# balazs-bamer/cdpr-simulation

Hardware: AMD Instinct MI355X
Metric: CDPR sim-steps/sec (whole node), 65 536 parallel 8-cable robots, 1 ms dt (higher is better)
Workload: dtype f32

## Files before the change

cdpr-simulation_amd/csrc/cdpr_onestep_kernel.hpp:

```cpp
#pragma once
#include "cdpr_step_kernel.hpp"

namespace cdpr {

CDPR_DEV void row_to_lds(const float4* src, float4* dst_row) {
  __builtin_amdgcn_global_load_lds((const __attribute__((address_space(1))) void*)src, (__attribute__((address_space(3))) void*)dst_row, 16, 0, 0);
}


template <int NP, bool PR = false, bool FULL = false>
CDPR_DEV void pid_pairs(const StepArgs& a, int calls, bool is_vel, const v2f (&desired)[NP], const v2f (&actual)[NP], const v2f (&win)[NP][kWin],
                        v2f (&ierr)[NP], v2f (&f)[NP], v2f (&e_new)[NP], float& dbg_p, float& dbg_i, float& dbg_d, bool is_force = false) {
  const PidCoef c = pid_coef<PR>(a, is_vel);
  const bool run = (!PR || calls != 0) && !is_force;
  const bool full = FULL || calls >= c.nbuf;
  const float (&wt)[kWin + 2] = a.wrow;
  v2f error[NP], acc[NP];
#pragma unroll
  for (int k = 0; k < NP; ++k) {
    error[k] = desired[k] - actual[k];
    acc[k] = splat(wt[kWin]) * error[k];
  }
#pragma unroll
  for (int j = 0; j < kWin; ++j) {
// ... 228 lines not shown
      ierr[2 * g] = (v2f){h.x, h.y};
      if (2 * g + 1 < NP) ierr[2 * g + 1] = (v2f){h.z, h.w};
    }
    const bool actual_is_vel = (a.flags & kFlagActualIsVelocity) != 0u;
    v2f actual[NP];
#pragma unroll
    for (int k = 0; k < NP; ++k) actual[k] = actual_is_vel ? qd[k] : q[k];
    const int ring_slot = a.ring_slot;
    pid_pairs<NP>(a, a.pid_calls, actual_is_vel, desired, actual, win, ierr, f, e_new, dbg_p, dbg_i, dbg_d);
    dbg_wrote = true;
    if (live) {
#pragma unroll
      for (int m = 0; m < 5; ++m) {
        if (m == (ring_slot >> 1)) {
#pragma unroll
          for (int k = 0; k < NP; ++k) CDPR_STORE_STATE(a.state, st, P + 5 * k + m, woff, ring_row(win[k], m, e_new[k], ring_slot));
        }
      }
#pragma unroll
      for (int g = 0; g < NH; ++g) {
        const int k1 = (2 * g + 1 < NP) ? 2 * g + 1 : 2 * g;
        CDPR_STORE_STATE(a.state, st, P + 5 * NP + g, woff, make_float4(ierr[2 * g].x, ierr[2 * g].y, ierr[k1].x, ierr[k1].y));
      }
    }
  }

  if (force_mode && !first_world) {
#pragma unroll
    for (int k = 0; k < NP; ++k) f[k] = desired[k];
  }

  if (PERSIST && more) {
    const uint32_t noff = nrr * 16u;
    if (run_pid) {
#pragma unroll
      for (int j = 0; j < kCtrl; ++j)
        row_to_lds(reinterpret_cast<const float4*>(reinterpret_cast<const char*>(a.state + (size_t)(P + j) * st) + noff), &stage[j][0]);
      if (kCmdLds) {
        const float* ncp = a.cmd + (size_t)nrr * N;
#pragma unroll
        for (int g = 0; g < kCmdRows; ++g) row_to_lds(reinterpret_cast<const float4*>(ncp) + g, &stage[kCtrl + g][0]);
      }
    }
  }

  CDPR_STAMP(5);
  v2f applied[NP];
  int td_flag = 0;
  if (TD) {
    v2f df[NP];
#pragma unroll
    for (int k = 0; k < NP; ++k) df[k] = f[k] - splat(a.td_mid);
    float g[6];
    if (FK) {
      jt_times<NP>(jest, df, g);
      normal_solve<NP, false>(jest, 0.f, g);
    } else {
      jt_times<NP>(jac, df, g);
      normal_solve<NP, false>(jac, 0.f, g);
    }
#pragma unroll
    for (int k = 0; k < NP; ++k) {
      v2f t = splat(a.td_mid);
#pragma unroll
      for (int c = 0; c < 6; ++c) t = fma2(g[c], FK ? jest[k][c] : jac[k][c], t);
      const v2f tc = max2(min2(t, splat(a.td_max)), splat(a.td_min));
      td_flag |= (tc.x != t.x) ? 1 : 0;
      if (2 * k + 1 < N) td_flag |= (tc.y != t.y) ? 1 : 0;
      applied[k] = tc;
    }
  } else {
#pragma unroll
    for (int k = 0; k < NP; ++k) applied[k] = f[k];
  }
  setforce_limits<NP>(a, qd, applied);

  if (a.dbg && live) write_pid_topic(a.dbg + (size_t)r * 9, dbg_wrote, dbg_wrote, dbg_p, dbg_i, dbg_d, desired[0].x, applied[0].x);
  if (publish && live) {
    store_slot(a.obs, st, 3, woff, make_float4(s.wz, fk_res, (float)fk_it, pack_flags(td_flag, travel_mask<N>(a, q))));
#pragma unroll
    for (int g = 0; g < G; ++g) {
      const int k0 = 2 * g, k1 = (2 * g + 1 < NP) ? 2 * g + 1 : 2 * g;
      const bool has = (2 * g + 1 < NP);
      store_slot(a.obs, st, 4 + 2 * G + g, woff,
                make_float4(applied[k0].x, applied[k0].y, has ? applied[k1].x : 0.f, has ? applied[k1].y : 0.f));
    }
  }

  CDPR_STAMP(6);
  {
    v2f tens[NP];
#pragma unroll
    for (int k = 0; k < NP; ++k) {
      tens[k] = fma2(-a.damping, qd[k], applied[k]);
      if (a.unilateral) tens[k] = max2(tens[k], splat(0.f));
    }
    if (FK) {
      uint32_t again = 0;
      asm volatile("" : "+v"(again));
      v2f len2[NP], l02[NP];
      ik_pairs<N, false>(lds + again, s.px, s.py, s.pz, s.qx, s.qy, s.qz, s.qw, len2, jac, l02);
    }
    float w[6];
    jt_times<NP>(jac, tens, w);
    w[0] = a.fgx - w[0];
    w[1] = a.fgy - w[1];
    w[2] = a.fgz - w[2];
    w[3] = -w[3];
    w[4] = -w[4];
    w[5] = -w[5];
    integrate(a, s, w);
  }
  if (PERSIST && more) {
    constexpr int kDmaOps = kCtrl + kCmdRows;
    static_assert(kDmaOps < 64, "vmcnt is a 6-bit counter");
    if (run_pid)
      __builtin_amdgcn_s_waitcnt(vmcnt_imm(kDmaOps));
    else
      __builtin_amdgcn_s_waitcnt(vmcnt_imm(0));
    asm volatile("" : "+a"(n0), "+a"(n1), "+a"(n2), "+a"(n3), "+a"(n4));
  }
  if (live) {
    CDPR_STORE_STATE(a.state, st, 0, woff, make_float4(s.px, s.py, s.pz, s.qx));
    CDPR_STORE_STATE(a.state, st, 1, woff, make_float4(s.qy, s.qz, s.qw, s.vx));
    CDPR_STORE_STATE(a.state, st, 2, woff, make_float4(s.vy, s.vz, s.wx, s.wy));
    CDPR_STORE_STATE(a.state, st, 3, woff, make_float4(s.wz, fkx, fky, fkz));
    if (FK) CDPR_STORE_STATE(a.state, st, 4, woff, make_float4(fkqx, fkqy, fkqz, fkqw));
  }
  CDPR_STAMP(7);
  if (!(PERSIST && more)) break;
  blk = nblk;
  r = nr;
  rr = nrr;
  live = r < a.batch;
  off = rr * 16u, woff = r * 16u;
  p0 = make_float4(n0.x, n0.y, n0.z, n0.w), p1 = make_float4(n1.x, n1.y, n1.z, n1.w), p2 = make_float4(n2.x, n2.y, n2.z, n2.w);
  p3 = make_float4(n3.x, n3.y, n3.z, n3.w), p4 = make_float4(n4.x, n4.y, n4.z, n4.w);
  staged = run_pid;
  }
}

#ifndef CDPR_CTL_LOAD_DELAY
#define CDPR_CTL_LOAD_DELAY 8
#endif
#ifndef CDPR_SPLIT_PRIO
#define CDPR_SPLIT_PRIO 1
#endif
#ifndef CDPR_STEADY_SHARED_IK
#define CDPR_STEADY_SHARED_IK 1
#endif
#ifndef CDPR_STEADY_NEWTON_WRITTEN_OUT
#define CDPR_STEADY_NEWTON_WRITTEN_OUT 1
#endif
constexpr int kIkRows = 7;
#ifdef CDPR_STAMPS
#define CDPR_SPLIT_STAMP(i)                                                                                          \
  do {                                                                                                               \
    __builtin_amdgcn_sched_barrier(0);                                                                               \
    if (a.stamps && lane == 0) a.stamps[(size_t)blockIdx.x * 8 + (i)] = __builtin_amdgcn_s_memrealtime();           \
    __builtin_amdgcn_sched_barrier(0);                                                                               \
  } while (0)
#else
#define CDPR_SPLIT_STAMP(i) do { } while (0)
#endif
#if defined(CDPR_STAMPS) && defined(CDPR_STAMPS_ITER)
#define CDPR_CTL_STAMP(i) do { } while (0)
#else
#define CDPR_CTL_STAMP(i) CDPR_SPLIT_STAMP(i)
#endif

template <int N, int XS, int ES, bool RAISED = true, bool STEADY = false>
CDPR_DEV void split_estimator_wave(const StepArgs& a, float* geo, float gval, uint32_t lane, bool live, size_t st, uint32_t off, uint32_t woff,
                                   const float4& p0, const float4& p1, const float4& p3, const v2f* x_force, v2f* x_tension, float* x_est,
                                   v2f* x_ik = nullptr) {
  constexpr int NP = cable_pairs(N);
#if defined(CDPR_STAMPS) && defined(CDPR_STAMPS_CLOCK)
  const unsigned long long clk0 = __builtin_amdgcn_s_memtime();
#endif
#if CDPR_SPLIT_PRIO == 1 || CDPR_SPLIT_PRIO == 4
  if (RAISED) __builtin_amdgcn_s_setprio(3);
#elif CDPR_SPLIT_PRIO == 3 || CDPR_SPLIT_PRIO == 5
  if (RAISED) __builtin_amdgcn_s_setprio(2);
#endif
  const float4 p4 = load_slot(a.state, st, 4, off);
  if (lane < NP * kGeomFloatsPerPair) geo[lane] = gval;
  __builtin_amdgcn_fence(__ATOMIC_RELEASE, "wavefront");
  __builtin_amdgcn_wave_barrier();
  __builtin_amdgcn_fence(__ATOMIC_ACQUIRE, "wavefront");
  float fkx = p3.y, fky = p3.z, fkz = p3.w, fkqx = p4.x, fkqy = p4.y, fkqz = p4.z, fkqw = p4.w;
  v2f len[NP];
  {
    v2f jac[NP][6], l0[NP];
    ik_pairs<N, false>(geo, p0.x, p0.y, p0.z, p0.w, p1.x, p1.y, p1.z, len, jac, l0);
    if (STEADY && CDPR_STEADY_SHARED_IK) {
#pragma unroll
      for (int k = 0; k < NP; ++k) {
        x_ik[(kIkRows * k) * 64 + lane] = len[k];
#pragma unroll
        for (int c = 0; c < 6; ++c) x_ik[(kIkRows * k + 1 + c) * 64 + lane] = jac[k][c];
      }
      __builtin_amdgcn_fence(__ATOMIC_RELEASE, "workgroup");
      __builtin_amdgcn_s_waitcnt(0xC07F);
      __builtin_amdgcn_s_barrier();
    }
  }
  float fk_res = 0.f;
  int fk_it = 0;
  v2f jest[NP][6];
  {
    v2f elen[NP], unused[NP];
    if (STEADY && CDPR_STEADY_NEWTON_WRITTEN_OUT) {
#pragma unroll
      for (int it = 0; it < 4; ++it) {
        ik_pairs<N, false>(geo, fkx, fky, fkz, fkqx, fkqy, fkqz, fkqw, elen, jest, unused);
        v2f res[NP];
#pragma unroll
        for (int k = 0; k < NP; ++k) res[k] = len[k] - elen[k];
        float g[6];
        jt_times<NP>(jest, res, g);
        normal_solve<NP>(jest, a.fk_lambda, g);
        fkx += g[0];
        fky += g[1];
        fkz += g[2];
        quat_apply_rotvec(fkqx, fkqy, fkqz, fkqw, g[3], g[4], g[5]);
#ifdef CDPR_STAMPS_ITER
        if (it < 3) {
          asm volatile("" ::"v"(fkqw));
          __builtin_amdgcn_sched_barrier(0);
          if (a.stamps && lane == 0) a.stamps[(size_t)blockIdx.x * 8 + 4 + it] = __builtin_amdgcn_s_memrealtime();
          __builtin_amdgcn_sched_barrier(0);
        }
#endif
      }
      fk_it = 4;
    } else {
      bool active = true;
      for (int it = 0; it < a.fk_iters; ++it) {
        ik_pairs<N, false>(geo, fkx, fky, fkz, fkqx, fkqy, fkqz, fkqw, elen, jest, unused);
        v2f res[NP];
        v2f rm = splat(0.f);
#pragma unroll
        for (int k = 0; k < NP; ++k) {
          res[k] = len[k] - elen[k];
          rm = max2(rm, abs2(res[k]));
        }
        active = active && !(fmaxf(rm.x, rm.y) < a.fk_tol);
        float g[6];
        jt_times<NP>(jest, res, g);
        normal_solve<NP>(jest, a.fk_lambda, g);
        if (active) {
          fkx += g[0];
          fky += g[1];
          fkz += g[2];
          quat_apply_rotvec(fkqx, fkqy, fkqz, fkqw, g[3], g[4], g[5]);
          ++fk_it;
        }
#ifdef CDPR_STAMPS_ITER
        if (it < 3) {
          asm volatile("" ::"v"(fkqw));
          __builtin_amdgcn_sched_barrier(0);
          if (a.stamps && lane == 0) a.stamps[(size_t)blockIdx.x * 8 + 4 + it] = __builtin_amdgcn_s_memrealtime();
          __builtin_amdgcn_sched_barrier(0);
        }
#endif
      }
    }
    ik_pairs<N, false>(geo, fkx, fky, fkz, fkqx, fkqy, fkqz, fkqw, elen, jest, unused);
    v2f rm = splat(0.f);
#pragma unroll
    for (int k = 0; k < NP; ++k) rm = max2(rm, abs2(len[k] - elen[k]));
    fk_res = fmaxf(rm.x, rm.y);
  }
  if (live) store_slot_aux<CDPR_SPLIT_PLAT_AUX>(a.state, st, 4, woff, make_float4(fkqx, fkqy, fkqz, fkqw));
  CDPR_SPLIT_STAMP(1);
  v2f td_l[6][3];
  float td_invd[6];
  normal_matrix_pk<NP, false>(jest, 0.f, td_l);
  chol_factor_pk(td_l, td_invd);
  __builtin_amdgcn_s_waitcnt(0xC07F);
  __builtin_amdgcn_s_barrier();
  CDPR_SPLIT_STAMP(2);
  __builtin_amdgcn_fence(__ATOMIC_ACQUIRE, "workgroup");
  v2f f[NP], df[NP], t_out[NP];
#pragma unroll
  for (int k = 0; k < NP; ++k) {
    f[k] = x_force[k * XS + lane];
    df[k] = f[k] - splat(a.td_mid);
  }
  int td_flag = 0;
  {
    float g[6];
    jt_times<NP>(jest, df, g);
    chol_apply_pk(td_l, td_invd, g);
#pragma unroll
    for (int k = 0; k < NP; ++k) {
      v2f t = splat(a.td_mid);
#pragma unroll
      for (int c = 0; c < 6; ++c) t = fma2(g[c], jest[k][c], t);
      const v2f tc = max2(min2(t, splat(a.td_max)), splat(a.td_min));
      td_flag |= (tc.x != t.x) ? 1 : 0;
      if (2 * k + 1 < N) td_flag |= (tc.y != t.y) ? 1 : 0;
      t_out[k] = tc;
    }
  }
#pragma unroll
  for (int k = 0; k < NP; ++k) x_tension[k * XS + lane] = t_out[k];
  x_est[0 * ES + lane] = fkx;
  x_est[1 * ES + lane] = fky;
  x_est[2 * ES + lane] = fkz;
  x_est[3 * ES + lane] = fk_res;
  x_est[4 * ES + lane] = (float)fk_it;
  x_est[5 * ES + lane] = (float)td_flag;
  __builtin_amdgcn_fence(__ATOMIC_RELEASE, "workgroup");
  __builtin_amdgcn_s_waitcnt(0xC07F);
  CDPR_SPLIT_STAMP(3);
#if defined(CDPR_STAMPS) && defined(CDPR_STAMPS_CLOCK)
  if (a.stamps && lane == 0) a.stamps[(size_t)blockIdx.x * 8 + 7] = __builtin_amdgcn_s_memtime() - clk0;
#endif
  __builtin_amdgcn_s_barrier();
}

template <int N, bool PR, bool STEADY, bool VEL>
CDPR_DEV void split_controller_wave(const StepArgs& a, float* geo, float gval, uint32_t lane, uint32_t r, uint32_t rr, bool live, size_t st, uint32_t off,
                                    uint32_t woff, const float4& p0, const float4& p1, const float4& p2, const float4& p3, v2f* x_force, const v2f* x_tension,
                                    const float* x_est, const v2f* x_ik = nullptr) {
  static_assert(!(STEADY && PR), "the steady instantiation serves uniform handles");
  constexpr int NP = cable_pairs(N);
  constexpr int P = plat_slots(true);
  constexpr int G = joint_groups(N);
  constexpr int NH = (NP + 1) / 2;
#if CDPR_SPLIT_PRIO == 2 || CDPR_SPLIT_PRIO == 5
  __builtin_amdgcn_s_setprio(3);
#endif
#if CDPR_CTL_LOAD_DELAY > 0
  __builtin_amdgcn_s_sleep(CDPR_CTL_LOAD_DELAY);
#endif
  float4 wraw[NP][5], hraw[NH];
#pragma unroll
  for (int k = 0; k < NP; ++k) {
#pragma unroll
    for (int m = 0; m < 5; ++m) wraw[k][m] = load_slot(a.state, st, P + 5 * k + m, off);
  }
#pragma unroll
  for (int g = 0; g < NH; ++g) hraw[g] = load_slot(a.state, st, P + 5 * NP + g, off);
  v2f desired[NP];
#pragma unroll
  for (int k = 0; k < NP; ++k) desired[k] = splat(0.f);
  const float* cp = a.cmd + (size_t)rr * N;
  if (N % 4 == 0) {
#pragma unroll
    for (int g = 0; g < N / 4; ++g) {
      const float4 v = reinterpret_cast<const float4*>(cp)[g];
      desired[2 * g] = (v2f){v.x, v.y};
      desired[2 * g + 1] = (v2f){v.z, v.w};
    }
  } else {
#pragma unroll
    for (int i = 0; i < N; ++i) {
      if (i & 1)
        desired[i / 2].y = cp[i];
      else
        desired[i / 2].x = cp[i];
    }
  }
  if (lane < NP * kGeomFloatsPerPair) geo[lane] = gval;
  __builtin_amdgcn_fence(__ATOMIC_RELEASE, "wavefront");
  __builtin_amdgcn_wave_barrier();
  __builtin_amdgcn_fence(__ATOMIC_ACQUIRE, "wavefront");

  Platform s;
  unpack_platform(p0, p1, p2, p3.x, s);

  v2f len[NP], q[NP], qd[NP], jac[NP][6];
  {
    v2f l0[NP];
    if (STEADY && CDPR_STEADY_SHARED_IK) {
      __builtin_amdgcn_s_barrier();
      __builtin_amdgcn_fence(__ATOMIC_ACQUIRE, "workgroup");
#pragma unroll
      for (int k = 0; k < NP; ++k) {
        len[k] = x_ik[(kIkRows * k) * 64 + lane];
#pragma unroll
        for (int c = 0; c < 6; ++c) jac[k][c] = x_ik[(kIkRows * k + 1 + c) * 64 + lane];
        l0[k] = *reinterpret_cast<const v2f*>(geo + k * kGeomFloatsPerPair + 12);
      }
    } else {
      ik_pairs<N, true>(geo, s.px, s.py, s.pz, s.qx, s.qy, s.qz, s.qw, len, jac, l0);
    }
#pragma unroll
    for (int k = 0; k < NP; ++k) {
      q[k] = l0[k] - len[k];
      qd[k] = -fma2(s.wz, jac[k][5], fma2(s.wy, jac[k][4], fma2(s.wx, jac[k][3],
                    fma2(s.vz, jac[k][2], fma2(s.vy, jac[k][1], splat(s.vx) * jac[k][0])))));
    }
  }
  const bool publish = STEADY || (a.publish_mask & 1ull) != 0ull;
  if (publish && live) {
    store_slot(a.obs, st, 0, woff, make_float4(s.px, s.py, s.pz, s.qx));
    store_slot(a.obs, st, 1, woff, make_float4(s.qy, s.qz, s.qw, s.vx));
    store_slot(a.obs, st, 2, woff, make_float4(s.vy, s.vz, s.wx, s.wy));
#pragma unroll
    for (int g = 0; g < G; ++g) {
      const int k0 = 2 * g, k1 = (2 * g + 1 < NP) ? 2 * g + 1 : 2 * g;
      const bool has = (2 * g + 1 < NP);
      store_slot(a.obs, st, 4 + g, woff, make_float4(q[k0].x, q[k0].y, has ? q[k1].x : 0.f, has ? q[k1].y : 0.f));
      store_slot(a.obs, st, 4 + G + g, woff, make_float4(qd[k0].x, qd[k0].y, has ? qd[k1].x : 0.f, has ? qd[k1].y : 0.f));
    }
  }

  v2f f[NP], e_new[NP], ierr[NP];
#pragma unroll
  for (int k = 0; k < NP; ++k) {
    f[k] = splat(0.f);
    e_new[k] = splat(0.f);
    ierr[k] = (k & 1) ? (v2f){hraw[k / 2].z, hraw[k / 2].w} : (v2f){hraw[k / 2].x, hraw[k / 2].y};
  }
  float dbg_p = 0.f, dbg_i = 0.f, dbg_d = 0.f;
  bool dbg_wrote = false;
  const bool first_world = !STEADY && (a.flags & kFlagFirstWorldStep) != 0u;
  uint32_t meta = 0u;
  if (PR) meta = a.meta[rr];
  const int calls = PR ? (int)(meta >> kMetaCallShift) : a.pid_calls;
  if (PR && live && !first_world) a.meta[r] = (uint8_t)((meta & kMetaModeMask) | ((uint32_t)min(calls + 1, (int)kMetaCallMax) << kMetaCallShift));
  const bool force_mode = !STEADY && !PR && (a.flags & kFlagForceMode) != 0u;
  if (force_mode && !first_world) {
#pragma unroll
    for (int k = 0; k < NP; ++k) f[k] = desired[k];
  } else if (STEADY || (!first_world && (PR || calls != 0))) {
    v2f win[NP][kWin];
#pragma unroll
    for (int k = 0; k < NP; ++k) {
#pragma unroll
      for (int m = 0; m < 5; ++m) {
        win[k][2 * m] = (v2f){wraw[k][m].x, wraw[k][m].y};
        win[k][2 * m + 1] = (v2f){wraw[k][m].z, wraw[k][m].w};
      }
    }
    const bool actual_is_vel = STEADY ? VEL : PR ? ((meta & kMetaModeMask) == kMetaVelocity) : ((a.flags & kFlagActualIsVelocity) != 0u);
    v2f actual[NP];
#pragma unroll
    for (int k = 0; k < NP; ++k) actual[k] = actual_is_vel ? qd[k] : q[k];
    const int ring_slot = a.ring_slot;
    const bool is_force = PR && (meta & kMetaModeMask) == kMetaForce;
#if CDPR_SPLIT_PRIO == 3 || CDPR_SPLIT_PRIO == 4
    __builtin_amdgcn_s_setprio(3);
#endif
    pid_pairs<NP, PR, STEADY>(a, calls, actual_is_vel, desired, actual, win, ierr, f, e_new, dbg_p, dbg_i, dbg_d, is_force);
    dbg_wrote = (!PR || calls != 0) && !is_force;
    if (live) {
#pragma unroll
      for (int m = 0; m < 5; ++m) {
        if (m == (ring_slot >> 1)) {
          if (!STEADY) {
#pragma unroll
            for (int k = 0; k < NP; ++k) CDPR_STORE_STATE(a.state, st, P + 5 * k + m, woff, ring_row(win[k], m, e_new[k], ring_slot));
          } else if (ring_slot & 1) {
#pragma unroll
            for (int k = 0; k < NP; ++k) CDPR_STORE_STATE(a.state, st, P + 5 * k + m, woff, make_float4(win[k][2 * m].x, win[k][2 * m].y, e_new[k].x, e_new[k].y));
          } else {
#pragma unroll
            for (int k = 0; k < NP; ++k) CDPR_STORE_STATE(a.state, st, P + 5 * k + m, woff, make_float4(e_new[k].x, e_new[k].y, win[k][2 * m + 1].x, win[k][2 * m + 1].y));
          }
        }
      }
#pragma unroll
      for (int g = 0; g < NH; ++g) {
        const int k1 = (2 * g + 1 < NP) ? 2 * g + 1 : 2 * g;
        CDPR_STORE_STATE(a.state, st, P + 5 * NP + g, woff, make_float4(ierr[2 * g].x, ierr[2 * g].y, ierr[k1].x, ierr[k1].y));
      }
    }
  }
#pragma unroll
  for (int k = 0; k < NP; ++k) x_force[k * 64 + lane] = f[k];
  __builtin_amdgcn_fence(__ATOMIC_RELEASE, "workgroup");
  __builtin_amdgcn_s_waitcnt(0xC07F);
  CDPR_CTL_STAMP(4);
#if CDPR_SPLIT_PRIO >= 3
  __builtin_amdgcn_s_setprio(0);
#endif
  __builtin_amdgcn_s_barrier();
  __builtin_amdgcn_s_barrier();
  CDPR_CTL_STAMP(5);
  __builtin_amdgcn_fence(__ATOMIC_ACQUIRE, "workgroup");
  v2f applied[NP];
#pragma unroll
  for (int k = 0; k < NP; ++k) applied[k] = x_tension[k * 64 + lane];
  const float fkx = x_est[0 * 64 + lane], fky = x_est[1 * 64 + lane], fkz = x_est[2 * 64 + lane], fk_res = x_est[3 * 64 + lane],
              fk_it = x_est[4 * 64 + lane], td_flag = x_est[5 * 64 + lane];
  setforce_limits<NP>(a, qd, applied);
  if (!STEADY && a.dbg && live) write_pid_topic(a.dbg + (size_t)r * 9, dbg_wrote, dbg_wrote, dbg_p, dbg_i, dbg_d, desired[0].x, applied[0].x);
  if (publish && live) {
    store_slot(a.obs, st, 3, woff, make_float4(s.wz, fk_res, fk_it, (!STEADY && a.travel_on) ? pack_flags((int)td_flag, travel_mask<N>(a, q)) : td_flag));
#pragma unroll
    for (int g = 0; g < G; ++g) {
      const int k0 = 2 * g, k1 = (2 * g + 1 < NP) ? 2 * g + 1 : 2 * g;
      const bool has = (2 * g + 1 < NP);
      store_slot(a.obs, st, 4 + 2 * G + g, woff,
                 make_float4(applied[k0].x, applied[k0].y, has ? applied[k1].x : 0.f, has ? applied[k1].y : 0.f));
    }
  }
  {
    v2f tens[NP];
#pragma unroll
    for (int k = 0; k < NP; ++k) {
      tens[k] = fma2(-a.damping, qd[k], applied[k]);
      if (a.unilateral) tens[k] = max2(tens[k], splat(0.f));
    }
    float w[6];
    jt_times<NP>(jac, tens, w);
    w[0] = a.fgx - w[0];
    w[1] = a.fgy - w[1];
    w[2] = a.fgz - w[2];
    w[3] = -w[3];
    w[4] = -w[4];
    w[5] = -w[5];
    integrate(a, s, w);
  }
  if (live) {
    store_slot_aux<CDPR_SPLIT_PLAT_AUX>(a.state, st, 0, woff, make_float4(s.px, s.py, s.pz, s.qx));
    store_slot_aux<CDPR_SPLIT_PLAT_AUX>(a.state, st, 1, woff, make_float4(s.qy, s.qz, s.qw, s.vx));
    store_slot_aux<CDPR_SPLIT_PLAT_AUX>(a.state, st, 2, woff, make_float4(s.vy, s.vz, s.wx, s.wy));
    store_slot_aux<CDPR_SPLIT_PLAT_AUX>(a.state, st, 3, woff, make_float4(s.wz, fkx, fky, fkz));
  }
  CDPR_CTL_STAMP(6);
}

template <int N, bool PR, bool STEADY, bool VEL>
CDPR_DEV void split_kernel_body(const StepArgs& a) {
  constexpr int NP = cable_pairs(N);
  __shared__ __attribute__((aligned(16))) float lds[2][NP * kGeomFloatsPerPair];
  __shared__ v2f x_force[NP][64];
  __shared__ v2f x_tension[NP][64];
  __shared__ float x_est[6][64];
  v2f* x_ik = nullptr;
  if constexpr (STEADY && CDPR_STEADY_SHARED_IK) {
    __shared__ v2f ik_rows_at_state[kIkRows * NP][64];
    x_ik = &ik_rows_at_state[0][0];
  }

  const uint32_t swap = __builtin_popcount(blockIdx.x & a.split_swap) & 1u;
  const uint32_t wave = (threadIdx.x >> 6) ^ swap, lane = threadIdx.x & 63u;
  const uint32_t r = blockIdx.x * 64u + lane;
  const uint32_t rr = (r < a.batch) ? r : (a.batch - 1u);
  const bool live = r < a.batch;
  const size_t st = a.stride;
  const uint32_t off = rr * 16u, woff = r * 16u;
  float* const geo = lds[wave];

  if (wave == 0) CDPR_SPLIT_STAMP(0);
#ifdef CDPR_STAMPS
  if (a.stamps && lane == 0)
    reinterpret_cast<uint32_t*>(&a.stamps[(size_t)blockIdx.x * 8 + 7])[threadIdx.x >> 6] =
        (__builtin_amdgcn_s_getreg((16 - 1) << 11 | 4) & 0xffffu) | ((__builtin_amdgcn_s_getreg((4 - 1) << 11 | 20) & 0xfu) << 16);
#endif
  const float gval = (lane < NP * kGeomFloatsPerPair) ? a.geom[lane] : 0.f;
  const float4 p0 = load_slot(a.state, st, 0, off), p1 = load_slot(a.state, st, 1, off), p2 = load_slot(a.state, st, 2, off),
               p3 = load_slot(a.state, st, 3, off);
  if (wave == 0) {
    split_estimator_wave<N, 64, 64, true, STEADY>(a, geo, gval, lane, live, st, off, woff, p0, p1, p3, &x_force[0][0], &x_tension[0][0], &x_est[0][0], x_ik);
    return;
  }
  split_controller_wave<N, PR, STEADY, VEL>(a, geo, gval, lane, r, rr, live, st, off, woff, p0, p1, p2, p3, &x_force[0][0], &x_tension[0][0], &x_est[0][0], x_ik);
}
template <int N, bool PR = false>
__global__ __launch_bounds__(128, 2) void cdpr_split_kernel(const StepArgs a) { split_kernel_body<N, PR, false, false>(a); }
template <int N, bool VEL>
__global__ __launch_bounds__(128, 2) void cdpr_split_steady_kernel(const StepArgs a) { split_kernel_body<N, false, true, VEL>(a); }

}
```

cdpr-simulation_amd/csrc/cdpr_step_kernel.hpp:

```cpp
#pragma once
#include <hip/hip_runtime.h>
#include <stdint.h>

namespace cdpr {

constexpr int kMaxCables = 8;
constexpr int kWin = 10;
constexpr int kGeomFloatsPerPair = 16;

typedef float v2f __attribute__((ext_vector_type(2)));

enum StepFlags : uint32_t {
  kFlagFirstWorldStep = 1u << 0,
  kFlagRolloutResetPid = 1u << 1,
  kFlagActualIsVelocity = 1u << 2,
  kFlagPublishAll = 1u << 4,
  kFlagForceMode = 1u << 3,
};

struct PidSet {
  float kf, kp, ki, kd, inv_ki, imax, imin, cmax, cmin;
  int clamp_cmd;
};

// ... 234 lines not shown
    for (int i = j + 1; i < 6; ++i) {
      float s = m[i][j];
#pragma unroll
      for (int k = 0; k < j; ++k) s = fmaf(-m[i][k], m[j][k], s);
      m[i][j] = s * invd[j];
    }
  }
#pragma unroll
  for (int i = 0; i < 6; ++i) {
    float s = g[i];
#pragma unroll
    for (int k = 0; k < i; ++k) s = fmaf(-m[i][k], g[k], s);
    g[i] = s * invd[i];
  }
#pragma unroll
  for (int i = 5; i >= 0; --i) {
    float s = g[i];
#pragma unroll
    for (int k = i + 1; k < 6; ++k) s = fmaf(-m[k][i], g[k], s);
    g[i] = s * invd[i];
  }
}

#ifndef CDPR_CHOL_PACKED
#define CDPR_CHOL_PACKED 1
#endif

CDPR_DEV void chol_factor_pk(v2f (&mp)[6][3], float (&invd)[6]) {
#pragma unroll
  for (int j = 0; j < 6; ++j) {
    const int p0 = j / 2;
    invd[j] = __frsqrt_rn((j & 1) ? mp[j][p0].y : mp[j][p0].x);
#pragma unroll
    for (int p = p0; p < 3; ++p) mp[j][p] = mp[j][p] * splat(invd[j]);
#pragma unroll
    for (int c = j + 1; c < 6; ++c) {
      const float lcj = (c & 1) ? mp[j][c / 2].y : mp[j][c / 2].x;
#pragma unroll
      for (int p = c / 2; p < 3; ++p) mp[c][p] = fma2(-lcj, mp[j][p], mp[c][p]);
    }
  }
}

CDPR_DEV void chol_apply_pk(const v2f (&mp)[6][3], const float (&invd)[6], float (&g)[6]) {
  v2f gp[3] = {(v2f){g[0], g[1]}, (v2f){g[2], g[3]}, (v2f){g[4], g[5]}};
#pragma unroll
  for (int j = 0; j < 6; ++j) {
    g[j] = ((j & 1) ? gp[j / 2].y : gp[j / 2].x) * invd[j];
#pragma unroll
    for (int p = (j + 1) / 2; p < 3; ++p) gp[p] = fma2(-g[j], mp[j][p], gp[p]);
  }
#pragma unroll
  for (int i = 5; i >= 0; --i) {
    float s = g[i];
#pragma unroll
    for (int k = i + 1; k < 6; ++k) s = fmaf(-((k & 1) ? mp[i][k / 2].y : mp[i][k / 2].x), g[k], s);
    g[i] = s * invd[i];
  }
}

CDPR_DEV void chol_solve_pk(v2f (&mp)[6][3], float (&g)[6]) {
  float invd[6];
  chol_factor_pk(mp, invd);
  chol_apply_pk(mp, invd, g);
}

template <int NP, bool LAMBDA = true>
CDPR_DEV void normal_matrix_pk(const v2f (&jac)[NP][6], float lambda, v2f (&mp)[6][3]) {
  v2f acc[21];
  gram_partial<NP>(jac, acc);
#pragma unroll
  for (int a = 0, e = 0; a < 6; ++a) {
#pragma unroll
    for (int b = 0; b <= a; ++b, ++e) {
      const float v = (LAMBDA && a == b) ? hsum(acc[e]) + lambda : hsum(acc[e]);
      if (a & 1)
        mp[b][a / 2].y = v;
      else
        mp[b][a / 2].x = v;
    }
  }
  mp[1][0].x = 0.f;
  mp[3][1].x = 0.f;
  mp[5][2].x = 0.f;
}

template <int NP, bool LAMBDA = true>
CDPR_DEV void normal_solve(const v2f (&jac)[NP][6], float lambda, float (&g)[6]) {
#if CDPR_CHOL_PACKED
  v2f mp[6][3];
  normal_matrix_pk<NP, LAMBDA>(jac, lambda, mp);
  chol_solve_pk(mp, g);
#else
  v2f acc[21];
  gram_partial<NP>(jac, acc);
  float m[6][6];
#pragma unroll
  for (int a = 0, e = 0; a < 6; ++a) {
#pragma unroll
    for (int b = 0; b <= a; ++b, ++e) m[a][b] = (LAMBDA && a == b) ? hsum(acc[e]) + lambda : hsum(acc[e]);
  }
  chol_solve(m, g);
#endif
}

struct PidCoef {
  float kf, kp, ki, kd, inv_ki, imax, imin, cmax, cmin;
  int nbuf;
  bool clamp;
};
template <bool PR>
CDPR_DEV PidCoef pid_coef(const StepArgs& a, bool is_vel) {
  PidCoef c;
  const bool alt = PR && !is_vel;
  c.kf = alt ? a.alt.kf : a.kf;
  c.kp = alt ? a.alt.kp : a.kp;
  c.ki = alt ? a.alt.ki : a.ki;
  c.kd = alt ? a.alt.kd : a.kd;
  c.inv_ki = alt ? a.alt.inv_ki : a.inv_ki;
  c.imax = alt ? a.alt.imax : a.imax;
  c.imin = alt ? a.alt.imin : a.imin;
  c.cmax = alt ? a.alt.cmax : a.cmax;
  c.cmin = alt ? a.alt.cmin : a.cmin;
  c.nbuf = a.nbuf;
  c.clamp = (alt ? a.alt.clamp_cmd : a.clamp_cmd) != 0;
  return c;
}
constexpr uint32_t kMetaModeMask = 3u, kMetaCallShift = 2u, kMetaCallMax = 63u;
constexpr uint32_t kMetaForce = 0u, kMetaPosition = 1u, kMetaVelocity = 2u;

struct Platform {
  float px, py, pz, qx, qy, qz, qw;
  float vx, vy, vz, wx, wy, wz;
};

CDPR_DEV void integrate_pose(const StepArgs& a, Platform& s);
CDPR_DEV void integrate_velocity(const StepArgs& a, Platform& s, const float (&w)[6]) {
  const Rot r = quat_to_rot(s.qx, s.qy, s.qz, s.qw);
  s.vx = fmaf(a.dt_inv_mass, w[0], s.vx);
  s.vy = fmaf(a.dt_inv_mass, w[1], s.vy);
  s.vz = fmaf(a.dt_inv_mass, w[2], s.vz);
  float tbx = fmaf(r.r20, w[5], fmaf(r.r10, w[4], r.r00 * w[3]));
  float tby = fmaf(r.r21, w[5], fmaf(r.r11, w[4], r.r01 * w[3]));
  float tbz = fmaf(r.r22, w[5], fmaf(r.r12, w[4], r.r02 * w[3]));
  const float obx = fmaf(r.r20, s.wz, fmaf(r.r10, s.wy, r.r00 * s.wx));
  const float oby = fmaf(r.r21, s.wz, fmaf(r.r11, s.wy, r.r01 * s.wx));
  const float obz = fmaf(r.r22, s.wz, fmaf(r.r12, s.wy, r.r02 * s.wx));
  const float iox = fmaf(a.ib[4], obz, fmaf(a.ib[3], oby, a.ib[0] * obx));
  const float ioy = fmaf(a.ib[5], obz, fmaf(a.ib[1], oby, a.ib[3] * obx));
  const float ioz = fmaf(a.ib[2], obz, fmaf(a.ib[5], oby, a.ib[4] * obx));
  tbx -= fmaf(oby, ioz, -(obz * ioy));
  tby -= fmaf(obz, iox, -(obx * ioz));
  tbz -= fmaf(obx, ioy, -(oby * iox));
  const float abx = fmaf(a.ibinv[4], tbz, fmaf(a.ibinv[3], tby, a.ibinv[0] * tbx));
  const float aby = fmaf(a.ibinv[5], tbz, fmaf(a.ibinv[1], tby, a.ibinv[3] * tbx));
  const float abz = fmaf(a.ibinv[2], tbz, fmaf(a.ibinv[5], tby, a.ibinv[4] * tbx));
  s.wx = fmaf(a.dt, fmaf(r.r02, abz, fmaf(r.r01, aby, r.r00 * abx)), s.wx);
  s.wy = fmaf(a.dt, fmaf(r.r12, abz, fmaf(r.r11, aby, r.r10 * abx)), s.wy);
  s.wz = fmaf(a.dt, fmaf(r.r22, abz, fmaf(r.r21, aby, r.r20 * abx)), s.wz);
}

CDPR_DEV void integrate_pose(const StepArgs& a, Platform& s) {
  s.px = fmaf(a.dt, s.vx, s.px);
  s.py = fmaf(a.dt, s.vy, s.py);
  s.pz = fmaf(a.dt, s.vz, s.pz);
  const float h = a.half_dt;
  const float nx = fmaf(h, fmaf(-s.wz, s.qy, fmaf(s.wy, s.qz, s.qw * s.wx)), s.qx);
  const float ny = fmaf(h, fmaf(-s.wx, s.qz, fmaf(s.wz, s.qx, s.qw * s.wy)), s.qy);
  const float nz = fmaf(h, fmaf(-s.wy, s.qx, fmaf(s.wx, s.qy, s.qw * s.wz)), s.qz);
  const float nw = fmaf(-h, fmaf(s.wz, s.qz, fmaf(s.wy, s.qy, s.wx * s.qx)), s.qw);
  const float inv = __frsqrt_rn(fmaf(nw, nw, fmaf(nz, nz, fmaf(ny, ny, nx * nx))));
  s.qx = nx * inv;
  s.qy = ny * inv;
  s.qz = nz * inv;
  s.qw = nw * inv;
}

CDPR_DEV void integrate(const StepArgs& a, Platform& s, const float (&w)[6]) {
  integrate_velocity(a, s, w);
  integrate_pose(a, s);
}

template <int N>
CDPR_DEV uint32_t travel_mask(const StepArgs& a, const v2f (&q)[cable_pairs(N)]) {
  uint32_t m = 0u;
  if (a.travel_on) {
#pragma unroll
    for (int k = 0; k < cable_pairs(N); ++k) {
      m |= (q[k].x < a.travel_lo || q[k].x > a.travel_hi) ? (1u << (2 * k)) : 0u;
      if (2 * k + 1 < N) m |= (q[k].y < a.travel_lo || q[k].y > a.travel_hi) ? (1u << (2 * k + 1)) : 0u;
    }
  }
  return m;
}
CDPR_DEV float pack_flags(int td_flag, uint32_t limit_mask) { return (float)((uint32_t)td_flag | (limit_mask << 1)); }

template <int N>
CDPR_DEV void apply_travel_stop(const StepArgs& a, Platform& s, const v2f (&q)[cable_pairs(N)], const v2f (&jac)[cable_pairs(N)][6]) {
  const Rot r = quat_to_rot(s.qx, s.qy, s.qz, s.qw);
  float vx = s.vx, vy = s.vy, vz = s.vz, wx = s.wx, wy = s.wy, wz = s.wz;
  for (int sweep = 0; sweep < a.travel_stop; ++sweep)
#pragma unroll
  for (int i = 0; i < N; ++i) {
    const int k = i / 2;
    float j[6];
#pragma unroll
    for (int c = 0; c < 6; ++c) j[c] = (i & 1) ? jac[k][c].y : jac[k][c].x;
    const float qi = (i & 1) ? q[k].y : q[k].x;
    const float qdn = -fmaf(j[5], wz, fmaf(j[4], wy, fmaf(j[3], wx, fmaf(j[2], vz, fmaf(j[1], vy, j[0] * vx)))));
    const bool hit = (qi >= a.travel_hi && qdn > 0.f) || (qi <= a.travel_lo && qdn < 0.f);
    const float tbx = fmaf(r.r20, j[5], fmaf(r.r10, j[4], r.r00 * j[3]));
    const float tby = fmaf(r.r21, j[5], fmaf(r.r11, j[4], r.r01 * j[3]));
    const float tbz = fmaf(r.r22, j[5], fmaf(r.r12, j[4], r.r02 * j[3]));
    const float abx = fmaf(a.ibinv[4], tbz, fmaf(a.ibinv[3], tby, a.ibinv[0] * tbx));
    const float aby = fmaf(a.ibinv[5], tbz, fmaf(a.ibinv[1], tby, a.ibinv[3] * tbx));
    const float abz = fmaf(a.ibinv[2], tbz, fmaf(a.ibinv[5], tby, a.ibinv[4] * tbx));
    const float awx = fmaf(r.r02, abz, fmaf(r.r01, aby, r.r00 * abx));
    const float awy = fmaf(r.r12, abz, fmaf(r.r11, aby, r.r10 * abx));
    const float awz = fmaf(r.r22, abz, fmaf(r.r21, aby, r.r20 * abx));
    const float d = fmaf(j[5], awz, fmaf(j[4], awy, fmaf(j[3], awx, fmaf(j[2], j[2], fmaf(j[1], j[1], j[0] * j[0])) * a.inv_mass)));
    const float lam = hit ? qdn / d : 0.f;
    const float lm = lam * a.inv_mass;
    vx = fmaf(lm, j[0], vx);
    vy = fmaf(lm, j[1], vy);
    vz = fmaf(lm, j[2], vz);
    wx = fmaf(lam, awx, wx);
    wy = fmaf(lam, awy, wy);
    wz = fmaf(lam, awz, wz);
  }
  s.vx = vx, s.vy = vy, s.vz = vz, s.wx = wx, s.wy = wy, s.wz = wz;
}

template <int N>
CDPR_DEV void integrate_lumped_velocity(const StepArgs& a, const float* lds, Platform& s, const v2f (&jac)[cable_pairs(N)][6],
                                        const v2f (&len)[cable_pairs(N)], float (&w)[6]) {
  constexpr int NP = cable_pairs(N);
  const Rot r = quat_to_rot(s.qx, s.qy, s.qz, s.qw);
  v2f fx = splat(0.f), fy = splat(0.f), fz = splat(0.f), tx = splat(0.f), ty = splat(0.f), tz = splat(0.f);
  v2f sa = splat(0.f), sax = splat(0.f), say = splat(0.f), saz = splat(0.f);
  v2f ixx = splat(0.f), iyy = splat(0.f), izz = splat(0.f), ixy = splat(0.f), ixz = splat(0.f), iyz = splat(0.f);
  v2f gram[21];
#pragma unroll
  for (int e = 0; e < 21; ++e) gram[e] = splat(0.f);
#pragma unroll
  for (int k = 0; k < NP; ++k) {
    const float4 g1 = *reinterpret_cast<const float4*>(lds + k * kGeomFloatsPerPair + 4);
    const float4 g2 = *reinterpret_cast<const float4*>(lds + k * kGeomFloatsPerPair + 8);
    const float4 g3 = *reinterpret_cast<const float4*>(lds + k * kGeomFloatsPerPair + 12);
    const v2f mask = ((N & 1) && k == NP - 1) ? (v2f){g3.z, g3.w} : splat(1.f);
    const v2f bx = {g1.z, g1.w}, by = {g2.x, g2.y}, bz = {g2.z, g2.w};
    const v2f rbx = fma2(r.r02, bz, fma2(r.r01, by, splat(r.r00) * bx));
    const v2f rby = fma2(r.r12, bz, fma2(r.r11, by, splat(r.r10) * bx));
    const v2f rbz = fma2(r.r22, bz, fma2(r.r21, by, splat(r.r20) * bx));
    const v2f ux = jac[k][0], uy = jac[k][1], uz = jac[k][2];
    const v2f l = (mask.x == 0.f || mask.y == 0.f) ? (v2f){len[k].x + (1.f - mask.x), len[k].y + (1.f - mask.y)} : len[k];
    const v2f il = (v2f){__frcp_rn(l.x), __frcp_rn(l.y)};
    const v2f vpx = fma2(s.wy, rbz, fma2(-s.wz, rby, splat(s.vx)));
    const v2f vpy = fma2(s.wz, rbx, fma2(-s.wx, rbz, splat(s.vy)));
    const v2f vpz = fma2(s.wx, rby, fma2(-s.wy, rbx, splat(s.vz)));
    const v2f along = fma2(uz, vpz, fma2(uy, vpy, ux * vpx));
    const v2f vtx = fma2(-along, ux, vpx), vty = fma2(-along, uy, vpy), vtz = fma2(-along, uz, vpz);
    const v2f oux = fma2(s.wy, uz, -(splat(s.wz) * uy)), ouy = fma2(s.wz, ux, -(splat(s.wx) * uz)), ouz = fma2(s.wx, uy, -(splat(s.wy) * ux));
    const v2f uvx = fma2(uy, vpz, -(uz * vpy)), uvy = fma2(uz, vpx, -(ux * vpz)), uvz = fma2(ux, vpy, -(uy * vpx));
    const v2f cl = splat(-a.ph_c) * il * mask;
    const v2f two_il = il + il;
    const v2f fdx = cl * fma2(two_il, vtx, -oux), fdy = cl * fma2(two_il, vty, -ouy), fdz = cl * fma2(two_il, vtz, -ouz);
    const v2f pm = splat(a.ph_mpt) * mask;
    const v2f fax = fma2(a.gx, pm, fdx), fay = fma2(a.gy, pm, fdy), faz = fma2(a.gz, pm, fdz);
    fx += fax;
    fy += fay;
    fz += faz;
    const v2f cm = splat(a.ph_c) * mask;
    tx += fma2(rby, faz, -(rbz * fay)) + cm * fma2(uvx, il, splat(-s.wx));
    ty += fma2(rbz, fax, -(rbx * faz)) + cm * fma2(uvy, il, splat(-s.wy));
    tz += fma2(rbx, fay, -(rby * fax)) + cm * fma2(uvz, il, splat(-s.wz));
    const v2f mu = splat(a.ph_jleg) * il * il;
    const v2f alpha = (mu + splat(a.ph_mpt)) * mask, beta = (splat(a.ph_max) - mu) * mask;
    sa += alpha;
    sax = fma2(alpha, rbx, sax);
    say = fma2(alpha, rby, say);
    saz = fma2(alpha, rbz, saz);
    const v2f rb2 = fma2(rbz, rbz, fma2(rby, rby, rbx * rbx));
    ixx = fma2(alpha, fma2(-rbx, rbx, rb2), ixx);
    iyy = fma2(alpha, fma2(-rby, rby, rb2), iyy);
    izz = fma2(alpha, fma2(-rbz, rbz, rb2), izz);
    ixy = fma2(-alpha, rbx * rby, ixy);
    ixz = fma2(-alpha, rbx * rbz, ixz);
    iyz = fma2(-alpha, rby * rbz, iyz);
    v2f bj[6];
#pragma unroll
    for (int c = 0; c < 6; ++c) bj[c] = beta * jac[k][c];
#pragma unroll
    for (int p = 0, e = 0; p < 6; ++p) {
#pragma unroll
      for (int q = 0; q <= p; ++q, ++e) gram[e] = fma2(bj[p], jac[k][q], gram[e]);
    }
  }
  const float b00 = a.ib[0], b11 = a.ib[1], b22 = a.ib[2], b01 = a.ib[3], b02 = a.ib[4], b12 = a.ib[5];
  const float c00 = fmaf(r.r02, b02, fmaf(r.r01, b01, r.r00 * b00)), c01 = fmaf(r.r02, b12, fmaf(r.r01, b11, r.r00 * b01)), c02 = fmaf(r.r02, b22, fmaf(r.r01, b12, r.r00 * b02));
  const float c10 = fmaf(r.r12, b02, fmaf(r.r11, b01, r.r10 * b00)), c11 = fmaf(r.r12, b12, fmaf(r.r11, b11, r.r10 * b01)), c12 = fmaf(r.r12, b22, fmaf(r.r11, b12, r.r10 * b02));
  const float c20 = fmaf(r.r22, b02, fmaf(r.r21, b01, r.r20 * b00)), c21 = fmaf(r.r22, b12, fmaf(r.r21, b11, r.r20 * b01)), c22 = fmaf(r.r22, b22, fmaf(r.r21, b12, r.r20 * b02));
  const float w00 = fmaf(c02, r.r02, fmaf(c01, r.r01, c00 * r.r00)) + a.ph_iadd_total, w11 = fmaf(c12, r.r12, fmaf(c11, r.r11, c10 * r.r10)) + a.ph_iadd_total,
              w22 = fmaf(c22, r.r22, fmaf(c21, r.r21, c20 * r.r20)) + a.ph_iadd_total;
  const float w01 = fmaf(c02, r.r12, fmaf(c01, r.r11, c00 * r.r10)), w02 = fmaf(c02, r.r22, fmaf(c01, r.r21, c00 * r.r20)),
              w12 = fmaf(c12, r.r22, fmaf(c11, r.r21, c10 * r.r20));
  const float iox = fmaf(w02, s.wz, fmaf(w01, s.wy, w00 * s.wx)), ioy = fmaf(w12, s.wz, fmaf(w11, s.wy, w01 * s.wx)), ioz = fmaf(w22, s.wz, fmaf(w12, s.wy, w02 * s.wx));
// ... 591 lines not shown
```

Before: 6.883 billion.

## Overlap steady tail prep with barrier wait and move obs status store to estimator wave

In the steady split kernel, the estimator wave publishes the FK position to LDS before the tension solve. It computes the clamp flag after the final barrier and writes the obs status slot itself, which shrinks the x_est exchange to three rows. The controller wave precomputes the rotation matrix and gyroscopic term between its two barriers, so only the tension-dependent part of velocity integration remains after the tensions arrive. The aim is to take work off the critical path between the waves' barriers, at the cost of extra live registers pinned through empty asm statements and a changed obs slot layout (p3.x instead of s.wz).

```diff
diff --git a/cdpr-simulation_amd/csrc/cdpr_onestep_kernel.hpp b/cdpr-simulation_amd/csrc/cdpr_onestep_kernel.hpp
--- a/cdpr-simulation_amd/csrc/cdpr_onestep_kernel.hpp
+++ b/cdpr-simulation_amd/csrc/cdpr_onestep_kernel.hpp
@@ -404,6 +404,12 @@
 #ifndef CDPR_STEADY_NEWTON_WRITTEN_OUT
 #define CDPR_STEADY_NEWTON_WRITTEN_OUT 1
 #endif
+#ifndef CDPR_STEADY_TAIL_PREP
+#define CDPR_STEADY_TAIL_PREP 1
+#endif
+#ifndef CDPR_STEADY_PIN_FACTOR
+#define CDPR_STEADY_PIN_FACTOR 1
+#endif
 constexpr int kIkRows = 7;
 #ifdef CDPR_STAMPS
 #define CDPR_SPLIT_STAMP(i)                                                                                          \
@@ -524,11 +530,27 @@
     fk_res = fmaxf(rm.x, rm.y);
   }
   if (live) store_slot_aux<CDPR_SPLIT_PLAT_AUX>(a.state, st, 4, woff, make_float4(fkqx, fkqy, fkqz, fkqw));
+  if (STEADY) {
+    x_est[0 * ES + lane] = fkx;
+    x_est[1 * ES + lane] = fky;
+    x_est[2 * ES + lane] = fkz;
+  }
   CDPR_SPLIT_STAMP(1);
   v2f td_l[6][3];
   float td_invd[6];
   normal_matrix_pk<NP, false>(jest, 0.f, td_l);
   chol_factor_pk(td_l, td_invd);
+  if (STEADY) {
+#if CDPR_STEADY_PIN_FACTOR
+#pragma unroll
+    for (int j = 0; j < 6; ++j) {
+      asm volatile("" ::"v"(td_invd[j]));
+#pragma unroll
+      for (int p = (j + 1) / 2; p < 3; ++p) asm volatile("" ::"v"(td_l[j][p]));
+    }
+#endif
+    __builtin_amdgcn_fence(__ATOMIC_RELEASE, "workgroup");
+  }
   __builtin_amdgcn_s_waitcnt(0xC07F);
   __builtin_amdgcn_s_barrier();
   CDPR_SPLIT_STAMP(2);
@@ -540,6 +562,7 @@
     df[k] = f[k] - splat(a.td_mid);
   }
   int td_flag = 0;
+  v2f t_raw[NP];
   {
     float g[6];
     jt_times<NP>(jest, df, g);
@@ -550,19 +573,25 @@
 #pragma unroll
       for (int c = 0; c < 6; ++c) t = fma2(g[c], jest[k][c], t);
       const v2f tc = max2(min2(t, splat(a.td_max)), splat(a.td_min));
-      td_flag |= (tc.x != t.x) ? 1 : 0;
-      if (2 * k + 1 < N) td_flag |= (tc.y != t.y) ? 1 : 0;
+      if (STEADY) {
+        t_raw[k] = t;
+      } else {
+        td_flag |= (tc.x != t.x) ? 1 : 0;
+        if (2 * k + 1 < N) td_flag |= (tc.y != t.y) ? 1 : 0;
+      }
       t_out[k] = tc;
     }
   }
 #pragma unroll
   for (int k = 0; k < NP; ++k) x_tension[k * XS + lane] = t_out[k];
-  x_est[0 * ES + lane] = fkx;
-  x_est[1 * ES + lane] = fky;
-  x_est[2 * ES + lane] = fkz;
-  x_est[3 * ES + lane] = fk_res;
-  x_est[4 * ES + lane] = (float)fk_it;
-  x_est[5 * ES + lane] = (float)td_flag;
+  if (!STEADY) {
+    x_est[0 * ES + lane] = fkx;
+    x_est[1 * ES + lane] = fky;
+    x_est[2 * ES + lane] = fkz;
+    x_est[3 * ES + lane] = fk_res;
+    x_est[4 * ES + lane] = (float)fk_it;
+    x_est[5 * ES + lane] = (float)td_flag;
+  }
   __builtin_amdgcn_fence(__ATOMIC_RELEASE, "workgroup");
   __builtin_amdgcn_s_waitcnt(0xC07F);
   CDPR_SPLIT_STAMP(3);
@@ -570,6 +599,18 @@
   if (a.stamps && lane == 0) a.stamps[(size_t)blockIdx.x * 8 + 7] = __builtin_amdgcn_s_memtime() - clk0;
 #endif
   __builtin_amdgcn_s_barrier();
+  if (STEADY) {
+#if CDPR_SPLIT_PRIO == 1 || CDPR_SPLIT_PRIO == 3 || CDPR_SPLIT_PRIO == 4 || CDPR_SPLIT_PRIO == 5
+    if (RAISED) __builtin_amdgcn_s_setprio(0);
+#endif
+#pragma unroll
+    for (int k = 0; k < NP; ++k) {
+      asm volatile("" : "+v"(t_raw[k]));
+      td_flag |= (t_out[k].x != t_raw[k].x) ? 1 : 0;
+      if (2 * k + 1 < N) td_flag |= (t_out[k].y != t_raw[k].y) ? 1 : 0;
+    }
+    if (live) store_slot(a.obs, st, 3, woff, make_float4(p3.x, fk_res, (float)fk_it, (float)td_flag));
+  }
 }
 
 template <int N, bool PR, bool STEADY, bool VEL>
@@ -731,18 +772,35 @@
   __builtin_amdgcn_s_setprio(0);
 #endif
   __builtin_amdgcn_s_barrier();
+  float fkx = 0.f, fky = 0.f, fkz = 0.f, fk_res = 0.f, fk_it = 0.f, td_flag = 0.f;
+  WorldStepPrep prep{};
+  if (STEADY && CDPR_STEADY_TAIL_PREP) {
+    __builtin_amdgcn_fence(__ATOMIC_ACQUIRE, "workgroup");
+    fkx = x_est[0 * 64 + lane], fky = x_est[1 * 64 + lane], fkz = x_est[2 * 64 + lane];
+    asm volatile("" : "+v"(s.qx), "+v"(s.qy), "+v"(s.qz), "+v"(s.qw), "+v"(s.wx), "+v"(s.wy), "+v"(s.wz));
+    prep = world_step_prepare(a, s);
+    asm volatile("" ::"v"(prep.r.r00), "v"(prep.r.r01), "v"(prep.r.r02), "v"(prep.r.r10), "v"(prep.r.r11), "v"(prep.r.r12));
+    asm volatile("" ::"v"(prep.r.r20), "v"(prep.r.r21), "v"(prep.r.r22), "v"(prep.gx), "v"(prep.gy), "v"(prep.gz));
+    asm volatile("" ::"v"(fkx), "v"(fky), "v"(fkz));
+  }
   __builtin_amdgcn_s_barrier();
   CDPR_CTL_STAMP(5);
   __builtin_amdgcn_fence(__ATOMIC_ACQUIRE, "workgroup");
   v2f applied[NP];
 #pragma unroll
   for (int k = 0; k < NP; ++k) applied[k] = x_tension[k * 64 + lane];
-  const float fkx = x_est[0 * 64 + lane], fky = x_est[1 * 64 + lane], fkz = x_est[2 * 64 + lane], fk_res = x_est[3 * 64 + lane],
-              fk_it = x_est[4 * 64 + lane], td_flag = x_est[5 * 64 + lane];
+  if (STEADY && !CDPR_STEADY_TAIL_PREP) {
+    fkx = x_est[0 * 64 + lane], fky = x_est[1 * 64 + lane], fkz = x_est[2 * 64 + lane];
+    prep = world_step_prepare(a, s);
+  }
+  if (!STEADY)
+    fkx = x_est[0 * 64 + lane], fky = x_est[1 * 64 + lane], fkz = x_est[2 * 64 + lane], fk_res = x_est[3 * 64 + lane],
+    fk_it = x_est[4 * 64 + lane], td_flag = x_est[5 * 64 + lane];
   setforce_limits<NP>(a, qd, applied);
   if (!STEADY && a.dbg && live) write_pid_topic(a.dbg + (size_t)r * 9, dbg_wrote, dbg_wrote, dbg_p, dbg_i, dbg_d, desired[0].x, applied[0].x);
   if (publish && live) {
-    store_slot(a.obs, st, 3, woff, make_float4(s.wz, fk_res, fk_it, (!STEADY && a.travel_on) ? pack_flags((int)td_flag, travel_mask<N>(a, q)) : td_flag));
+    if (!STEADY)
+      store_slot(a.obs, st, 3, woff, make_float4(s.wz, fk_res, fk_it, a.travel_on ? pack_flags((int)td_flag, travel_mask<N>(a, q)) : td_flag));
 #pragma unroll
     for (int g = 0; g < G; ++g) {
       const int k0 = 2 * g, k1 = (2 * g + 1 < NP) ? 2 * g + 1 : 2 * g;
@@ -766,7 +824,12 @@
     w[3] = -w[3];
     w[4] = -w[4];
     w[5] = -w[5];
-    integrate(a, s, w);
+    if (STEADY) {
+      integrate_velocity_prepared(a, s, w, prep);
+      integrate_pose(a, s);
+    } else {
+      integrate(a, s, w);
+    }
   }
   if (live) {
     store_slot_aux<CDPR_SPLIT_PLAT_AUX>(a.state, st, 0, woff, make_float4(s.px, s.py, s.pz, s.qx));
@@ -783,7 +846,7 @@
   __shared__ __attribute__((aligned(16))) float lds[2][NP * kGeomFloatsPerPair];
   __shared__ v2f x_force[NP][64];
   __shared__ v2f x_tension[NP][64];
-  __shared__ float x_est[6][64];
+  __shared__ float x_est[STEADY ? 3 : 6][64];
   v2f* x_ik = nullptr;
   if constexpr (STEADY && CDPR_STEADY_SHARED_IK) {
     __shared__ v2f ik_rows_at_state[kIkRows * NP][64];
diff --git a/cdpr-simulation_amd/csrc/cdpr_step_kernel.hpp b/cdpr-simulation_amd/csrc/cdpr_step_kernel.hpp
--- a/cdpr-simulation_amd/csrc/cdpr_step_kernel.hpp
+++ b/cdpr-simulation_amd/csrc/cdpr_step_kernel.hpp
@@ -410,6 +410,44 @@
   tbx -= fmaf(oby, ioz, -(obz * ioy));
   tby -= fmaf(obz, iox, -(obx * ioz));
   tbz -= fmaf(obx, ioy, -(oby * iox));
+  const float abx = fmaf(a.ibinv[4], tbz, fmaf(a.ibinv[3], tby, a.ibinv[0] * tbx));
+  const float aby = fmaf(a.ibinv[5], tbz, fmaf(a.ibinv[1], tby, a.ibinv[3] * tbx));
+  const float abz = fmaf(a.ibinv[2], tbz, fmaf(a.ibinv[5], tby, a.ibinv[4] * tbx));
+  s.wx = fmaf(a.dt, fmaf(r.r02, abz, fmaf(r.r01, aby, r.r00 * abx)), s.wx);
+  s.wy = fmaf(a.dt, fmaf(r.r12, abz, fmaf(r.r11, aby, r.r10 * abx)), s.wy);
+  s.wz = fmaf(a.dt, fmaf(r.r22, abz, fmaf(r.r21, aby, r.r20 * abx)), s.wz);
+}
+
+struct WorldStepPrep {
+  Rot r;
+  float gx, gy, gz;
+};
+CDPR_DEV WorldStepPrep world_step_prepare(const StepArgs& a, const Platform& s) {
+  WorldStepPrep p;
+  p.r = quat_to_rot(s.qx, s.qy, s.qz, s.qw);
+  const Rot& r = p.r;
+  const float obx = fmaf(r.r20, s.wz, fmaf(r.r10, s.wy, r.r00 * s.wx));
+  const float oby = fmaf(r.r21, s.wz, fmaf(r.r11, s.wy, r.r01 * s.wx));
+  const float obz = fmaf(r.r22, s.wz, fmaf(r.r12, s.wy, r.r02 * s.wx));
+  const float iox = fmaf(a.ib[4], obz, fmaf(a.ib[3], oby, a.ib[0] * obx));
+  const float ioy = fmaf(a.ib[5], obz, fmaf(a.ib[1], oby, a.ib[3] * obx));
+  const float ioz = fmaf(a.ib[2], obz, fmaf(a.ib[5], oby, a.ib[4] * obx));
+  p.gx = fmaf(oby, ioz, -(obz * ioy));
+  p.gy = fmaf(obz, iox, -(obx * ioz));
+  p.gz = fmaf(obx, ioy, -(oby * iox));
+  return p;
+}
+CDPR_DEV void integrate_velocity_prepared(const StepArgs& a, Platform& s, const float (&w)[6], const WorldStepPrep& p) {
+  const Rot& r = p.r;
+  s.vx = fmaf(a.dt_inv_mass, w[0], s.vx);
+  s.vy = fmaf(a.dt_inv_mass, w[1], s.vy);
+  s.vz = fmaf(a.dt_inv_mass, w[2], s.vz);
+  float tbx = fmaf(r.r20, w[5], fmaf(r.r10, w[4], r.r00 * w[3]));
+  float tby = fmaf(r.r21, w[5], fmaf(r.r11, w[4], r.r01 * w[3]));
+  float tbz = fmaf(r.r22, w[5], fmaf(r.r12, w[4], r.r02 * w[3]));
+  tbx -= p.gx;
+  tby -= p.gy;
+  tbz -= p.gz;
   const float abx = fmaf(a.ibinv[4], tbz, fmaf(a.ibinv[3], tby, a.ibinv[0] * tbx));
   const float aby = fmaf(a.ibinv[5], tbz, fmaf(a.ibinv[1], tby, a.ibinv[3] * tbx));
   const float abz = fmaf(a.ibinv[2], tbz, fmaf(a.ibinv[5], tby, a.ibinv[4] * tbx));
```

Result: no change. 6.871 billion (-0.2%).
